# MuellerNico/DD2360-RayTracing

Measured on AMD Instinct MI355X. Metric: Msamples/s (W*H*spp/render_time) at 1200x800, 10000 spheres, higher is better.
Workload: dtype f32

## Files before the change

### dd2360-raytracing_amd/csrc/rt_kernels.hip

```cpp
#include <hip/hip_runtime.h>
#include <float.h>
#include "rt_device.h"
#include "rt_tuning.h"
#include "rt_sampling.h"

#ifdef RT_TU_CONTRACT
#pragma clang fp contract(fast)
#else
#pragma clang fp contract(off)
#endif

namespace rt {
#ifdef RT_TU_CONTRACT
namespace fmac {
#endif

#define RT_DEV static __device__ __forceinline__

#include "rt_stats.h"

struct Rng { uint32_t d, v0, v1, v2, v3, v4; };

RT_DEV float rng_uniform(Rng& s) {
    const uint32_t t = s.v0 ^ (s.v0 >> 2);
// ... 338 lines not shown
RT_DEV void walk_sync() { __builtin_amdgcn_fence(__ATOMIC_SEQ_CST, "wavefront"); __builtin_amdgcn_wave_barrier(); }
RT_DEV unsigned walk_excl_scan(unsigned v, unsigned& total) {
    int x = (int)v;
    x += __builtin_amdgcn_update_dpp(0, x, 0x111, 0xf, 0xf, false);
    x += __builtin_amdgcn_update_dpp(0, x, 0x112, 0xf, 0xf, false);
    x += __builtin_amdgcn_update_dpp(0, x, 0x114, 0xf, 0xf, false);
    x += __builtin_amdgcn_update_dpp(0, x, 0x118, 0xf, 0xf, false);
    x += __builtin_amdgcn_update_dpp(0, x, 0x142, 0xa, 0xf, false);
    x += __builtin_amdgcn_update_dpp(0, x, 0x143, 0xc, 0xf, false);
    total = (unsigned)__builtin_amdgcn_readlane(x, 63);
    return (unsigned)x - v;
}

RT_DEV void pool_candidate_b(const DevTree& T, const float4* s_nodes, WalkLds& L, const uint4 c, const float4 blo, const float4 bhi STAT_ARG) {
    const int owner = (int)c.w;
    const float b = __uint_as_float(c.x), disc = __uint_as_float(c.y);
    const float4 r0 = L.ray[2 * owner], r1 = L.ray[2 * owner + 1];
    RayF q; q.o = {r0.x, r0.y, r0.z}; q.d = {r0.w, r1.x, r1.y};
    const float a = r1.z;
    const unsigned long long k0 = L.key[owner];
    const float best_t = __uint_as_float((unsigned)(k0 >> 32));
    const int best = (int)(unsigned)k0;
    const float sq = sqrtf(disc);
    float cand = __builtin_inff();
    const float t1 = (-b - sq) / a;
    if (t1 > 0.001f) cand = t1;
    else { const float t2 = (-b + sq) / a; if (t2 > 0.001f) cand = t2; }
    if (!(cand <= best_t)) return;
    const int id = __float_as_int(blo.w);
    STAT(st, ST_OFFERS, 1);
// ... 45 lines not shown
    const float f_atm = a * (0.001f * 0.9999f - 1e-6f);
    bool walking = W.walking && W.i != W.iend;
    const int nw0 = __popcll(__ballot(walking));
    L.ray[2 * lane] = make_float4(r.o.x, r.o.y, r.o.z, r.d.x);
    while (true) {
        L.ray[2 * lane + 1] = make_float4(r.d.y, r.d.z, a, __builtin_fmaf(a * best_t, 1.0001f, 1e-6f * a));
        L.key[lane] = ((unsigned long long)__float_as_uint(best_t) << 32) | (unsigned)best;
        if (lane == 0) { L.tie_lo = 0u; L.tie_hi = 0u; }
        walk_sync();
        const int cols_now = nw0 * RT_POOL_COLS_THIN <= kWalkPool ? RT_POOL_COLS_THIN : RT_POOL_COLS;
        int e0[RT_POOL_COLS_THIN], e1[RT_POOL_COLS_THIN];
#pragma unroll
        for (int c = 0; c < RT_POOL_COLS_THIN; ++c) {
            e0[c] = 0; e1[c] = 0;
            if (c < cols_now && walking && W.i != W.iend) {
                STAT(st, ST_COLS, 1);
                const float u0 = W.on_c + ((float)W.i - W.om_c) * W.slope, u1 = u0 + W.slope;
                const float lo = (fminf(u0, u1) - q_c) * fF, hi = (fmaxf(u0, u1) + q_c) * fF;
                if (hi >= 0.0f && lo < fGf) {
                    const int k0 = (int)fmaxf(lo, 0.0f), k1 = (int)fminf(hi, fGfm);
                    const unsigned cbase = (unsigned)(W.coff + W.i * Gf);
                    e0[c] = cs[cbase + (unsigned)k0]; e1[c] = cs[cbase + (unsigned)k1 + 1u];
                }
                W.i += step; ++W.cols;
            }
        }
        unsigned n_seg = 0u;
#pragma unroll
        for (int c = 0; c < RT_POOL_COLS_THIN; ++c) {
            if (c >= RT_POOL_COLS && c >= cols_now) break;
            const bool has = e1[c] > e0[c];
// ... 35 lines not shown
                    S.sg = (n_seg > 1u && p1 <= begin ? 1u : 0u) + (n_seg > 2u && p2 <= begin ? 1u : 0u) + (n_seg > 3u && p3 <= begin ? 1u : 0u);
                } else if (begin < S.end) {
                    unsigned lo = 0u, hi = n_seg;
#pragma unroll
                    for (int it = 0; it < 8; ++it) {
                        const unsigned mid = (lo + hi) >> 1;
                        if (hi - lo > 1u) { if (L.pref[mid] <= begin) lo = mid; else hi = mid; }
                    }
                    S.sg = lo;
                }
            }
            unsigned qn = 0u;
            if (RT_POOL_DIRECT && RT_POOL_SPANS == 1 && total <= 64u) {
                PoolSpan& S = sp[0];
                const bool act = S.cur < S.end;
                STAT(st, ST_A_ITERS_WAVE, 1);
                unsigned he = 0u;
                if (act) {
                    const uint2 sd = L.seg[S.sg];
                    const unsigned p0 = L.pref[S.sg];
                    he = sd.x - p0 + S.cur;
                    S.owner = (int)(sd.y >> 26);
                    const float4 r0 = L.ray[2 * S.owner], r1 = L.ray[2 * S.owner + 1];
                    S.q.o = {r0.x, r0.y, r0.z}; S.q.d = {r0.w, r1.x, r1.y}; S.a = r1.z; S.abt = r1.w;
                    S.atm = S.a * (0.001f * 0.9999f - 1e-6f);
                }
                const float4 s4 = hot[he], blo = A.brick[2 * he], bhi = A.brick[2 * he + 1];
                STAT(st, ST_TESTS, act ? 1 : 0); STAT(st, ST_A_LANE_STEPS, act ? 1 : 0);
                const float ocx = S.q.o.x - s4.x, ocy = S.q.o.y - s4.y, ocz = S.q.o.z - s4.z;
                const float b = ocx * S.q.d.x + ocy * S.q.d.y + ocz * S.q.d.z;
                const float c = (ocx * ocx + ocy * ocy + ocz * ocz) - s4.w;
                const float disc = b * b - S.a * c;
                const float ab = fabsf(b);
                const float Lm = __builtin_fmaf(ab, -1e-4f, -b) - S.abt, M = __builtin_fmaf(ab, -1e-4f, b) + S.atm;
                const float P = fmaxf(Lm, M);
                if (act && disc > 0.0f && !(P > 0.0f && P * P > disc * 1.0003f)) {
                    STAT(st, ST_DISCPOS, 1);
                    pool_candidate_b(T, s_nodes, L, make_uint4(__float_as_uint(b), __float_as_uint(disc), he, (unsigned)S.owner), blo, bhi STAT_PASS);
                }
            } else
            while (true) {
                bool any = false;
#pragma unroll
                for (int j = 0; j < RT_POOL_SPANS; ++j) any = any || sp[j].cur < sp[j].end;
                if (__ballot(any) == 0ull) break;
                STAT(st, ST_A_ITERS_WAVE, 1);
                bool act[RT_POOL_SPANS]; unsigned he[RT_POOL_SPANS]; float4 s4[RT_POOL_SPANS];
#pragma unroll
                for (int j = 0; j < RT_POOL_SPANS; ++j) {
                    PoolSpan& S = sp[j];
                    act[j] = S.cur < S.end;
                    if (act[j] && S.cur >= S.seg_end) {
                        const uint2 sd = L.seg[S.sg];
                        const unsigned p0 = L.pref[S.sg];
                        ++S.sg;
                        S.seg_end = p0 + (sd.y & 0x3ffffffu);
                        S.base = sd.x - p0;
                        const int ow = (int)(sd.y >> 26);
                        if (ow != S.owner) {
                            S.owner = ow;
                            const float4 r0 = L.ray[2 * ow], r1 = L.ray[2 * ow + 1];
// ... 11 lines not shown
                    const PoolSpan& S = sp[j];
                    STAT(st, ST_TESTS, act[j] ? 1 : 0); STAT(st, ST_A_LANE_STEPS, act[j] ? 1 : 0);
                    const float ocx = S.q.o.x - s4[j].x, ocy = S.q.o.y - s4[j].y, ocz = S.q.o.z - s4[j].z;
                    const float b = ocx * S.q.d.x + ocy * S.q.d.y + ocz * S.q.d.z;
                    const float c = (ocx * ocx + ocy * ocy + ocz * ocz) - s4[j].w;
                    const float disc = b * b - S.a * c;
                    const float ab = fabsf(b);
                    const float Lm = __builtin_fmaf(ab, -1e-4f, -b) - S.abt, M = __builtin_fmaf(ab, -1e-4f, b) + S.atm;
                    const float P = fmaxf(Lm, M);
                    hold[j] = act[j] && disc > 0.0f && !(P > 0.0f && P * P > disc * 1.0003f);
                    hb[j] = b; hd[j] = disc;
                    anyhold = anyhold || hold[j];
                    if (act[j]) ++sp[j].cur;
                }
                if (__ballot(anyhold) != 0ull) {
#pragma unroll
                    for (int j = 0; j < RT_POOL_SPANS; ++j) {
                        const unsigned long long hm = __ballot(hold[j]);
                        if (hm != 0ull) {
                            const unsigned slot = qn + __builtin_amdgcn_mbcnt_hi((unsigned)(hm >> 32), __builtin_amdgcn_mbcnt_lo((unsigned)hm, 0u));
                            if (hold[j]) {
                                STAT(st, ST_DISCPOS, 1);
                                const uint4 ce = make_uint4(__float_as_uint(hb[j]), __float_as_uint(hd[j]), he[j], (unsigned)sp[j].owner);
                                if (slot < (unsigned)kWalkCand) L.cq[slot] = ce;
                                else pool_candidate(T, s_nodes, L, ce STAT_PASS);
                            }
                            qn += (unsigned)__popcll(hm);
                        }
                    }
                }
                if (qn >= 64u) pool_drain(T, s_nodes, L, lane, qn STAT_PASS);
            }
            pool_drain(T, s_nodes, L, lane, qn STAT_PASS);
            (void)f_atm;
            const unsigned long long k = L.key[lane];
            best_t = __uint_as_float((unsigned)(k >> 32)); best = (int)(unsigned)k;
            const unsigned tmask = lane < 32 ? L.tie_lo : L.tie_hi;
            if ((tmask >> (lane & 31)) & 1u) tie = true;
        }
        if (walking && best >= 0) walk_clip(W, A, best_t);
        walking = walking && W.i != W.iend;
        const int left = __popcll(__ballot(walking));
        if (left == 0) break;
        if (RT_QUORUM_DEN > 0 && nw0 >= RT_QUORUM_MIN && left * RT_QUORUM_DEN <= nw0) break;
    }
    W.walking = walking;
}

template <int RT_QUORUM_DEN>
RT_DEV void walk_pool_dense(const DevTree& T, const float4* s_nodes, WalkLds& L, const RayF& r, float a, Walk& W, float& best_t, int& best, bool& tie STAT_ARG) {
    constexpr int PB = RT_DENSE_PB;
    const DevAccel& A = T.acc;
    const int32_t* __restrict__ cs = A.cs;
    const float4* __restrict__ hot = A.hot;
    const int lane = threadIdx.x & 63;
    const int Gf = A.Gf;
    const float fF = (float)A.F, fGf = (float)Gf, fGfm = fGf - 0.5f, q_c = A.rq_c;
    const int step = W.fwd ? 1 : -1;
    bool walking = W.walking && W.i != W.iend;
    const int nw0 = __popcll(__ballot(walking));
    L.ray[2 * lane] = make_float4(r.o.x, r.o.y, r.o.z, r.d.x);
    while (true) {
        L.ray[2 * lane + 1] = make_float4(r.d.y, r.d.z, a, __builtin_fmaf(a * best_t, 1.0001f, 1e-6f * a));
        L.key[lane] = ((unsigned long long)__float_as_uint(best_t) << 32) | (unsigned)best;
        if (lane == 0) { L.tie_lo = 0u; L.tie_hi = 0u; }
        walk_sync();
        int e0 = 0, e1 = 0;
        if (walking && W.i != W.iend) {
            STAT(st, ST_COLS, 1);
            const float u0 = W.on_c + ((float)W.i - W.om_c) * W.slope, u1 = u0 + W.slope;
            const float lo = (fminf(u0, u1) - q_c) * fF, hi = (fmaxf(u0, u1) + q_c) * fF;
            if (hi >= 0.0f && lo < fGf) {
                const int k0 = (int)fmaxf(lo, 0.0f), k1 = (int)fminf(hi, fGfm);
                const unsigned cbase = (unsigned)(W.coff + W.i * Gf);
                e0 = cs[cbase + (unsigned)k0]; e1 = cs[cbase + (unsigned)k1 + 1u];
            }
            W.i += step; ++W.cols;
        }
        const bool has = e1 > e0;
        const unsigned long long m = __ballot(has);
        const unsigned n_seg = (unsigned)__popcll(m);
        if (has) {
            const unsigned slot = __builtin_amdgcn_mbcnt_hi((unsigned)(m >> 32), __builtin_amdgcn_mbcnt_lo((unsigned)m, 0u));
            L.seg[slot] = make_uint2((unsigned)e0, (unsigned)(e1 - e0) | ((unsigned)lane << 26));
// ... 14 lines not shown
            S.end = min(begin + C, total); S.cur = begin; S.seg_end = begin; S.base = 0u; S.sg = 0u; S.owner = lane;
            S.q.o = {0.f, 0.f, 0.f}; S.q.d = {0.f, 1.f, 0.f}; S.a = 1.0f; S.abt = 0.0f; S.atm = 0.0f;
            if (begin < S.end) {
                unsigned lo = 0u, hi = n_seg;
#pragma unroll
                for (int it = 0; it < 6; ++it) {
                    const unsigned mid = (lo + hi) >> 1;
                    if (hi - lo > 1u) { if (L.pref[mid] <= begin) lo = mid; else hi = mid; }
                }
                S.sg = lo;
            }
            unsigned qn = 0u;
            while (true) {
                const bool act = S.cur < S.end;
                if (__ballot(act) == 0ull) break;
                STAT(st, ST_A_ITERS_WAVE, 1);
                if (act && S.cur >= S.seg_end) {
                    const uint2 sd = L.seg[S.sg];
                    const unsigned p0 = L.pref[S.sg];
                    ++S.sg;
                    S.seg_end = p0 + (sd.y & 0x3ffffffu);
                    S.base = sd.x - p0;
                    S.owner = (int)(sd.y >> 26);
                    const float4 r0 = L.ray[2 * S.owner], r1 = L.ray[2 * S.owner + 1];
                    S.q.o = {r0.x, r0.y, r0.z}; S.q.d = {r0.w, r1.x, r1.y}; S.a = r1.z;
                    S.atm = S.a * (0.001f * 0.9999f - 1e-6f);
                }
                const unsigned nb = act ? min((unsigned)PB, min(S.seg_end, S.end) - S.cur) : 0u;
                const unsigned he0 = act ? S.base + S.cur : 0u;
                const float4* __restrict__ hp = hot + he0;
                float4 s4[PB];
// ... 6 lines not shown
                bool anyhold = false;
#pragma unroll
                for (int k = 0; k < PB; ++k) {
                    const float ocx = S.q.o.x - s4[k].x, ocy = S.q.o.y - s4[k].y, ocz = S.q.o.z - s4[k].z;
                    const float b = ocx * S.q.d.x + ocy * S.q.d.y + ocz * S.q.d.z;
                    const float c = (ocx * ocx + ocy * ocy + ocz * ocz) - s4[k].w;
                    const float disc = b * b - S.a * c;
                    const float ab = fabsf(b);
                    const float Lm = __builtin_fmaf(ab, -1e-4f, -b) - S.abt, M = __builtin_fmaf(ab, -1e-4f, b) + S.atm;
                    const float P = fmaxf(Lm, M);
                    hold[k] = (unsigned)k < nb && disc > 0.0f && !(P > 0.0f && P * P > disc * 1.0003f);
                    hb[k] = b; hd[k] = disc;
                    anyhold = anyhold || hold[k];
                }
                if (__ballot(anyhold) != 0ull) {
#pragma unroll
                    for (int k = 0; k < PB; ++k) {
                        const unsigned long long hm = __ballot(hold[k]);
                        if (hm != 0ull) {
                            const unsigned slot = qn + __builtin_amdgcn_mbcnt_hi((unsigned)(hm >> 32), __builtin_amdgcn_mbcnt_lo((unsigned)hm, 0u));
                            if (hold[k]) {
                                STAT(st, ST_DISCPOS, 1);
                                const uint4 ce = make_uint4(__float_as_uint(hb[k]), __float_as_uint(hd[k]), he0 + (unsigned)k, (unsigned)S.owner);
                                if (slot < (unsigned)kWalkCand) L.cq[slot] = ce;
                                else pool_candidate(T, s_nodes, L, ce STAT_PASS);
                            }
                            qn += (unsigned)__popcll(hm);
                        }
                    }
                }
                S.cur += nb;
                if (qn >= (unsigned)RT_DENSE_DRAIN) pool_drain(T, s_nodes, L, lane, qn STAT_PASS);
            }
            pool_drain(T, s_nodes, L, lane, qn STAT_PASS);
            const unsigned long long k = L.key[lane];
            best_t = __uint_as_float((unsigned)(k >> 32)); best = (int)(unsigned)k;
            const unsigned tmask = lane < 32 ? L.tie_lo : L.tie_hi;
            if ((tmask >> (lane & 31)) & 1u) tie = true;
        }
        if (walking && best >= 0) walk_clip(W, A, best_t);
        walking = walking && W.i != W.iend;
        const int left = __popcll(__ballot(walking));
        if (left == 0) break;
        if (RT_QUORUM_DEN > 0 && nw0 >= RT_QUORUM_MIN && left * RT_QUORUM_DEN <= nw0) break;
    }
    W.walking = walking;
}

constexpr int kHotLarge = 8;
constexpr int kHotSlots = 1 + 3 * kHotLarge;
RT_DEV float4* hot_spheres(const float4* s_nodes, int n_nodes) { return (float4*)((WalkLds*)(s_nodes + n_nodes * 3) + 4); }
template <bool POOL>
RT_DEV void stage_tree_fp32(const DevScene& S, const DevTree& T, float4* s_nodes) {
    const int n4 = T.n_nodes * 3;
    for (int t = threadIdx.x; t < n4; t += 256) s_nodes[t] = T.nodes4[t];
    if (POOL) {
        float4* h = hot_spheres(s_nodes, T.n_nodes);
        const int nl = min(T.acc.n_large, kHotLarge);
        if (threadIdx.x == 0) h[0] = S.ground_valid ? S.list_hot[0] : make_float4(0.f, 0.f, 0.f, 0.f);
        if ((int)threadIdx.x < nl) h[1 + threadIdx.x] = T.acc.large_hot[threadIdx.x];
        if ((int)threadIdx.x < 2 * nl) h[1 + kHotLarge + threadIdx.x] = T.acc.large_brick[threadIdx.x];
    }
    __syncthreads();
}

struct TreeState { Walk W; float g_t; int g_id; bool tie, pending; unsigned work, cols; };
RT_DEV void tree_state_init(TreeState& ts) {
    ts.pending = false; ts.tie = false; ts.g_t = FLT_MAX; ts.g_id = -1; ts.work = 0u; ts.cols = 0u; ts.W.work = 0u; ts.W.cols = 0u;
    ts.W.walking = false; ts.W.i = 0; ts.W.iend = 0; ts.W.coff = 0; ts.W.om_c = 0.f; ts.W.on_c = 0.f; ts.W.slope = 0.f; ts.W.dm_c = 0.f; ts.W.fwd = true;
}

template <int COOPG>
RT_DEV void closest_tree(const DevScene& S, const DevTree& T, const float4* s_nodes, const RayF& r, float a, bool live, float& closest, int& best, TreeState& ts STAT_ARG) {
    const bool fresh = live && !ts.pending;
    STAT(st, ST_RAYS, fresh ? 1 : 0);
    if (fresh) { closest = FLT_MAX; best = -1; }
    if (S.ground_valid && fresh) {
        WPASS(WP_GROUND);
        const float4 g = COOPG != 1 ? hot_spheres(s_nodes, T.n_nodes)[0] : S.list_hot[0];
        int gb = -1;
        { const float ocx = r.o.x - g.x, ocy = r.o.y - g.y, ocz = r.o.z - g.z;
          const float b = ocx * r.d.x + ocy * r.d.y + ocz * r.d.z;
          const float c = (ocx * ocx + ocy * ocy + ocz * ocz) - g.w;
          if (__ballot(fresh && !(b > 0.0f && c > 0.0f)) != 0ull) sphere_test(r, a, g.x, g.y, g.z, g.w, 0, closest, gb); }
// ... 54 lines not shown
        }
        if (walker) {
            ts.pending = ts.W.walking;
            if (!ts.pending && ts.tie) { closest = ts.g_t; best = ts.g_id; slow = true; STAT(st, ST_TIE, 1); }
        }
    }
    RT_STATS_ONLY(
    const unsigned long long tS0 = TICK(); st.cyc[1] += tS0 - tG;
    )
    if (__ballot(slow) != 0ull) { WPASS(WP_SCAN); tree_scan(s_nodes, r, a, slow, closest, best); }
    RT_STATS_ONLY(
    st.cyc[3] += TICK() - tS0;
    )
}

RT_DEV V3 random_in_unit_sphere(Rng& s) {
    V3 p;
    do {
        WPASS(WP_REJ_ITER);
        const float x = rng_uniform(s); const float y = rng_uniform(s); const float z = rng_uniform(s);
        p.x = signed_unit(x); p.y = signed_unit(y); p.z = signed_unit(z);
    } while (p.x * p.x + p.y * p.y + p.z * p.z >= 1.0f);
    return p;
}

RT_DEV RayF primary_ray(const rt_camera& c, int i, int j, int max_x, int max_y, Rng& s) {
    const float u = ((float)i + rng_uniform(s)) / (float)max_x;
    const float v = ((float)j + rng_uniform(s)) / (float)max_y;
    float px, py;
    WPASS(WP_PRIMARY);
// ... 272 lines not shown
            fb[0] = (float)pix_iters; fb[1] = (float)((__builtin_amdgcn_s_memrealtime() >> 4) & 0xffffffull); fb[2] = (float)((pix_t0 >> 4) & 0xffffffull);
            )
        } else {
            if (A.ns == 1) { fb[0] = col.x; fb[1] = col.y; fb[2] = col.z; }
            else { fb[0] += col.x; fb[1] += col.y; fb[2] += col.z; }
        }
    };
    RT_STATS_ONLY(
    Stats st; for (int q = 0; q < ST_N; ++q) st.c[q] = 0;
    for (int q = 0; q < 8; ++q) st.cyc[q] = 0;
    const unsigned long long tK0 = TICK(), rK0 = __builtin_amdgcn_s_memrealtime();
    unsigned int dbg_thin_iters = 0, dbg_long = 0;
    unsigned long long th[4] = {0, 0, 0, 0};
    unsigned long long dbg_thin_cyc = 0, dbg_thin_closest = 0, dbg_thin1_cyc = 0; unsigned int dbg_thin1_iters = 0; unsigned long long dbg_t_prev = TICK();
    )
    constexpr bool kSolo = TREE && COOPG == 5;
    if (kSolo && lane == 0 && begin_long_pixel(true)) solo = true;
    if (__ballot(live) == 0ull && lane < RT_LONG_PER_WAVE) begin_long_pixel(false);
    if (__ballot(live) != 0ull) { thin = true; __builtin_amdgcn_s_setprio(3); }

    const unsigned int thin_cap = (unsigned int)(n_waves / RT_THIN_CAP_DEN);
    float closest = FLT_MAX; int best = -1;
    TreeState ts; tree_state_init(ts);
    while (true) {
        const unsigned long long m_live = __ballot(live);
        const unsigned long long m_long = __ballot(live && is_long);
        if (!thin && m_long != 0ull) {
            unsigned int prev = 0;
            if (lane == 0) prev = atomicAdd(cold_args()->queue + 1, 1u);
            prev = __builtin_amdgcn_readfirstlane(prev);
            if (prev < thin_cap) { thin = true; thin_counted = true; __builtin_amdgcn_s_setprio(3); }
            else { if (lane == 0) atomicSub(cold_args()->queue + 1, 1u); is_long = false; }
        } else if (thin && m_long == 0ull) {
// ... 29 lines not shown
        { const unsigned long long now = TICK(); const int nl2 = __popcll(__ballot(live));
          if (thin) { ++dbg_thin_iters; dbg_thin_cyc += now - dbg_t_prev; if (nl2 <= 2) { ++dbg_thin1_iters; dbg_thin1_cyc += now - dbg_t_prev; } }
          dbg_t_prev = now; }
        )
        RT_STATS_ONLY(
        { const int nl = __popcll(__ballot(live)); STAT(st, nl >= 56 ? ST_LIVE_GE56 : nl >= 32 ? ST_LIVE_32 : nl >= 8 ? ST_LIVE_8 : ST_LIVE_LT8, 1);
          WPASS_CLASS(nl >= 56 ? 0 : nl >= 32 ? 1 : nl >= 8 ? 2 : 3); }
        )
        const float a = dot3(r.d, r.d);
        if (!TREE) { closest = FLT_MAX; best = -1; }
        RT_STATS_ONLY(
        const unsigned long long tC0 = TICK();
        const unsigned long long c4_ = st.cyc[4], c5_ = st.cyc[5], c1_ = st.cyc[1], c3_ = st.cyc[3];
        const bool thin12 = thin && __popcll(__ballot(live)) <= 2;
        )
        if (TREE) closest_tree<COOPG>(A.scene, A.tree, s_nodes, r, a, live, closest, best, ts STAT_PASS);
        else closest_list(A.scene, r, a, live, closest, best);
        RT_STATS_ONLY(
        const unsigned long long tC1 = TICK(); st.cyc[0] += tC1 - tC0; st.cyc[2] += tC0; if (thin) dbg_thin_closest += tC1 - tC0;
        if (TREE && thin12) { th[0] += (st.cyc[4] - c4_) - tC0; th[1] += st.cyc[5] - c5_; th[2] += (st.cyc[1] - c1_) - (st.cyc[5] - c5_); th[3] += st.cyc[3] - c3_; }
        if (live) { ++pix_iters; }
        )
        if (live && !(TREE && ts.pending)) {
            ++iters;
            bool done;
            float lum = 0.0f;
            if (best >= 0) {
                const bool cont = scatter(cold_args()->scene, best, closest, r, att, s);
                ++depth;
                done = !cont || depth >= 50;
            } else {
// ... 18 lines not shown
                        RT_STATS_ONLY(
                        if (!is_long) ++dbg_long;
                        )
                        is_long = true;
                    }
                    else if (RT_MED_RATE > 0 && (sample & 7) == 0 && iters >= (unsigned int)(RT_MED_RATE * sample)) is_med = true;
                } else {
                    WPASS(WP_ENDPIX);
                    end_pixel();
                    RT_STATS_ONLY(
                    pix_iters = 0;
                    )
                    STAT(st, ST_SWITCHES, 1);
                    live = false; is_long = false; is_med = false;
                    if (kSolo && solo && begin_long_pixel(true)) {  }
                    else if (lane < RT_LONG_PER_WAVE && begin_long_pixel(false)) { solo = false;  }
                }
            }
        }
    }

    RT_STATS_ONLY(
    for (int q = 0; q < ST_N; ++q) {
        const bool wave_level = (q == ST_LOOP_ITERS_WAVE || (q >= ST_LIVE_GE56 && q <= ST_LIVE_LT8));
        const bool lane_max = (q == ST_A_ITERS_WAVE || q == ST_B_ROUNDS_WAVE);
        if (lane_max) { int m = (int)st.c[q]; for (int off = 32; off > 0; off >>= 1) m = max(m, __shfl_xor(m, off)); if (lane == 0) atomicAdd(&g_stats[q], (unsigned long long)m); }
        else if (st.c[q] && (!wave_level || lane == 0)) atomicAdd(&g_stats[q], (unsigned long long)st.c[q]);
    }
    { int nl = (int)dbg_long; for (int off = 32; off > 0; off >>= 1) nl += __shfl_xor(nl, off); dbg_long = (unsigned int)nl; }
    if (lane == 0) {
        const long long wv = (long long)blockIdx.x * 4 + (threadIdx.x >> 6);
// ... 401 lines not shown
    const unsigned int mine = s_bin[threadIdx.x];
    s_base[threadIdx.x] = mine != 0u ? start + atomicAdd(&ws[256 + threadIdx.x], mine) : 0u;
    __syncthreads();
#pragma unroll
    for (int u = 0; u < 4; ++u) {
        if (key[u] < 0) continue;
        const int sub = (int)((b0 + 256 * u + threadIdx.x) & 15);
        const unsigned int pos = s_base[key[u]] + local[u];
        const int lx = 2 * (sub & 3), ly = 2 * (sub >> 2);
#pragma unroll
        for (int q = 0; q < 4; ++q) tail_list[pos + q] = (unsigned int)(tile[u] * 64 + (ly + (q >> 1)) * 8 + lx + (q & 1));
    }
}
#endif

template <bool TREE, int COOPG>
RT_DEV void trace_record(const RenderArgs& A, const float4* s_nodes, const RayF& r, bool live, rt_hit_record* out) {
    const DevScene& S = A.scene; const DevTree& T = A.tree;
    const float a = dot3(r.d, r.d);
    float closest = FLT_MAX; int best = -1;
    RT_STATS_ONLY(
    Stats st; for (int q = 0; q < ST_N; ++q) st.c[q] = 0;
    for (int q = 0; q < 8; ++q) st.cyc[q] = 0;
    )
    if (TREE) {
        TreeState ts; tree_state_init(ts);
        bool act = live;
        do { closest_tree<COOPG>(S, T, s_nodes, r, a, act, closest, best, ts STAT_PASS); act = live && ts.pending; } while (__ballot(act) != 0ull);
    } else closest_list(S, r, a, live, closest, best);
    if (!live) return;
    rt_hit_record h;
    h.sphere = best; h.t = 0.f; h.p[0] = h.p[1] = h.p[2] = 0.f; h.normal[0] = h.normal[1] = h.normal[2] = 0.f;
    if (best >= 0) {
        const float4 g = S.geom[best];
        h.t = closest;
        h.p[0] = r.o.x + closest * r.d.x; h.p[1] = r.o.y + closest * r.d.y; h.p[2] = r.o.z + closest * r.d.z;
        h.normal[0] = (h.p[0] - g.x) / g.w; h.normal[1] = (h.p[1] - g.y) / g.w; h.normal[2] = (h.p[2] - g.z) / g.w;
    }
    *out = h;
}

template <bool TREE, int COOPG = 1>
__global__ __launch_bounds__(256) void k_trace(RenderArgs A, const float* rays, long long n, rt_hit_record* out) {
    extern __shared__ float4 s_nodes[];
    if (TREE) stage_tree_fp32<COOPG != 1>(A.scene, A.tree, s_nodes);
    const long long gid = (long long)blockIdx.x * 256 + threadIdx.x;
    const bool live = gid < n;
    RayF r; r.o = {0.f, 0.f, 0.f}; r.d = {0.f, 1.f, 0.f};
    if (live) { const float* p = rays + gid * 6; r.o = {p[0], p[1], p[2]}; r.d = {p[3], p[4], p[5]}; }
    trace_record<TREE, COOPG>(A, s_nodes, r, live, out + gid);
}

#ifndef RT_TU_CONTRACT
template <bool TREE, int COOPG = 1>
__global__ __launch_bounds__(256) void k_guides(RenderArgs A, long long n, rt_hit_record* out) {
    extern __shared__ float4 s_nodes[];
    if (TREE) stage_tree_fp32<COOPG != 1>(A.scene, A.tree, s_nodes);
    const long long gid = (long long)blockIdx.x * 256 + threadIdx.x;
    const bool live = gid < n;
    RayF r; r.o = {0.f, 0.f, 0.f}; r.d = {0.f, 1.f, 0.f};
    if (live) {
        const rt_camera& c = A.scene.cam;
        const int i = (int)(gid % A.max_x), j = (int)(gid / A.max_x);
        const float u = ((float)i + 0.5f) / (float)A.max_x;
        const float v = ((float)j + 0.5f) / (float)A.max_y;
// ... 267 lines not shown
    return hipGetLastError();
}
hipError_t launch_adapt_zero(unsigned int* p, int n, hipStream_t st) {
    if (n <= 0) return hipSuccess;
    hipLaunchKernelGGL(k_adapt_zero, dim3((unsigned)((n + 255) / 256)), dim3(256), 0, st, p, n);
    return hipGetLastError();
}
#endif

hipError_t launch_trace(const DevScene& S, const DevTree& T, bool tree, const float* rays, long long n, rt_hit_record* out, hipStream_t st) {
    if (n <= 0) return hipSuccess;
    const unsigned blocks = (unsigned)((n + 255) / 256);
    RenderArgs A{};
    A.scene = S; A.tree = T;
    if (!tree) return launch_trace_list(A, blocks, rays, n, out, st);
    if (render_variant(true, 0, T.acc) == 5) hipLaunchKernelGGL((k_trace<true, 5>), dim3(blocks), dim3(256), tree_lds_bytes(T.n_nodes, true), st, A, rays, n, out);
    else if (render_variant(true, 0, T.acc) == 4) hipLaunchKernelGGL((k_trace<true, 4>), dim3(blocks), dim3(256), tree_lds_bytes(T.n_nodes, true), st, A, rays, n, out);
    else if (render_variant(true, 0, T.acc) == 2) hipLaunchKernelGGL((k_trace<true, 2>), dim3(blocks), dim3(256), tree_lds_bytes(T.n_nodes, true), st, A, rays, n, out);
    else hipLaunchKernelGGL((k_trace<true>), dim3(blocks), dim3(256), tree_lds_bytes(T.n_nodes), st, A, rays, n, out);
    return hipGetLastError();
}

#ifndef RT_TU_CONTRACT
hipError_t launch_guides(const DevScene& S, const DevTree& T, bool tree, int max_x, int max_y, rt_hit_record* out, hipStream_t st) {
    const long long n = (long long)max_x * max_y;
    if (n <= 0) return hipSuccess;
    const unsigned blocks = (unsigned)((n + 255) / 256);
    RenderArgs A{};
    A.scene = S; A.tree = T; A.max_x = max_x; A.max_y = max_y;
    if (!tree) return launch_guides_list(A, blocks, n, out, st);
// ... 34 lines not shown
```

### dd2360-raytracing_amd/csrc/rt_stats.h

```cpp
#pragma once
#ifdef RT_STATS
enum { ST_RAYS, ST_FAST, ST_SLOW, ST_TIE, ST_COLS, ST_TESTS, ST_DISCPOS, ST_OFFERS, ST_ELIG, ST_ELIG_NODES, ST_A_ITERS_WAVE, ST_B_ROUNDS_WAVE,
       ST_LOOP_ITERS_WAVE, ST_A_LANE_STEPS, ST_B_LANES, ST_SAMPLES, ST_LIVE_GE56, ST_LIVE_32, ST_LIVE_8, ST_LIVE_LT8, ST_SWITCHES,
       ST_CYC_TOTAL, ST_CYC_CLOSEST, ST_CYC_WALK_A, ST_CYC_WALK_B, ST_CYC_SCAN, ST_CYC_SHADE, ST_REALTIME,
       ST_SPARE0, ST_SPARE1, ST_SPARE2, ST_SPARE3, ST_SPARE4, ST_SPARE5, ST_SPARE6,
       WP_GROUND, WP_LARGE_K, WP_LARGE_EXACT, WP_OFFER_NODE, WP_OFFER_RAYBOX, WP_ELIG_FN, WP_ELIG_LIST, WP_SETUP, WP_A_COL, WP_A_BATCH, WP_A_HOLD,
       WP_B_OFFER, WP_B_CLIP, WP_COOP_CHUNK, WP_SCAN, WP_SC_ANY, WP_SC_LAMB, WP_SC_METAL, WP_SC_DIEL, WP_REJ_ITER, WP_PRIMARY, WP_DISK_ITER, WP_SKY, WP_ENDPIX,
       TH_GROUND, TH_LARGE_SETUP, TH_WALK, TH_SCAN, ST_N };
#ifdef RT_STATS_LIGHT
#define TICK() 0ull
#else
#define TICK() ((unsigned long long)__builtin_amdgcn_s_memtime())
#endif
__device__ unsigned long long g_stats[ST_N];
__device__ int g_pilot_dbg[1 << 20];
__device__ unsigned long long g_wave_dbg[8192 * 4];
struct Stats { unsigned int c[ST_N]; unsigned long long cyc[8]; };
#ifdef RT_STATS_LIGHT
#define STAT(st, k, v) ((void)0)
#else
#define STAT(st, k, v) ((st).c[k] += (v))
#endif
constexpr int kWpBlocks = WP_ENDPIX - WP_GROUND + 1;
__device__ unsigned long long g_wp_cls[4 * kWpBlocks];
#ifdef RT_STATS_WPASS
__shared__ int s_wp_cls[4];
#define WPASS(k) do { const int l_ = (int)(threadIdx.x & 63); if (__builtin_amdgcn_readfirstlane(l_) == l_) { atomicAdd(&g_stats[k], 1ull); \
    atomicAdd(&g_wp_cls[(s_wp_cls[(threadIdx.x >> 6) & 3] & 3) * kWpBlocks + ((k) - WP_GROUND)], 1ull); } } while (0)
#define WPASS_CLASS(c) do { const int l_ = (int)(threadIdx.x & 63); if (__builtin_amdgcn_readfirstlane(l_) == l_) s_wp_cls[(threadIdx.x >> 6) & 3] = (c); } while (0)
#else
#define WPASS(k) ((void)0)
#define WPASS_CLASS(c) ((void)0)
#endif
#define STAT_ARG , Stats& st
#define STAT_PASS , st
#define RT_STATS_ONLY(...) __VA_ARGS__
#define RT_STATS_READERS \
hipError_t read_pilot_dbg(int* out, int n) { return hipMemcpyFromSymbol(out, HIP_SYMBOL(g_pilot_dbg), sizeof(int) * (size_t)(n < (1 << 20) ? n : (1 << 20))); } \
hipError_t read_wave_dbg(unsigned long long* out) { return hipMemcpyFromSymbol(out, HIP_SYMBOL(g_wave_dbg), sizeof(unsigned long long) * 8192 * 4); } \
hipError_t read_wp_classes(unsigned long long* out, int reset) { \
    hipError_t e = hipMemcpyFromSymbol(out, HIP_SYMBOL(g_wp_cls), sizeof(unsigned long long) * 4 * kWpBlocks); \
    if (e != hipSuccess) return e; \
    if (reset) { unsigned long long z[4 * kWpBlocks] = {0}; e = hipMemcpyToSymbol(HIP_SYMBOL(g_wp_cls), z, sizeof(z)); } \
// ... 18 lines not shown
```

### dd2360-raytracing_amd/csrc/rt_tuning.h

```cpp
#pragma once

#ifndef RT_RENDER_WAVES
#define RT_RENDER_WAVES 4
#endif

#ifndef RT_LONG_RATE
#define RT_LONG_RATE 14
#endif
#ifndef RT_LONG_RATE_DENSE
#define RT_LONG_RATE_DENSE 20
#endif
#ifndef RT_LONG_CHECK
#define RT_LONG_CHECK 4
#endif
#ifndef RT_F_INFLIGHT
#define RT_F_INFLIGHT 1.35f
#endif
#ifndef RT_F_INFLIGHT_DENSE
#define RT_F_INFLIGHT_DENSE 1.1f
#endif

#ifndef RT_F_STATIC
#define RT_F_STATIC 1.07f
#endif
// ... 20 lines not shown
#endif
#ifndef RT_LONG_RATE_MIN
#define RT_LONG_RATE_MIN 8
#endif
#ifndef RT_PILOT_LONG_SUM_MIN
#define RT_PILOT_LONG_SUM_MIN 120
#endif
#ifndef RT_MED_RATE
#define RT_MED_RATE 12
#endif
#ifndef RT_THIN_CAP_DEN
#define RT_THIN_CAP_DEN 4
#endif
#ifndef RT_LONG_PER_WAVE
#define RT_LONG_PER_WAVE 16
#endif
#ifndef RT_PILOT_SAMPLES
#define RT_PILOT_SAMPLES 2
#endif
#ifndef RT_PILOT_LONG_SUM
#define RT_PILOT_LONG_SUM 200
#endif
#ifndef RT_SOLO_DENSITY
#define RT_SOLO_DENSITY 1.0
#endif
#ifndef RT_PILOT_SOLO_SUM
#define RT_PILOT_SOLO_SUM 200
#endif
#ifndef RT_PILOT_CAP
#define RT_PILOT_CAP 35
// ... 97 lines not shown
```

Baseline: 4592.

## Add quad-lane cooperative ground and large-sphere tests for sparse long-pixel waves

When a wave has at most 16 live rays, all on lanes that are multiples of four, each ray's three idle neighbour lanes now test the ground and the first three large spheres in parallel, and the results are reduced with DPP quad broadcasts. Long-pixel chains are placed on lanes 0,4,...,60 so this layout arises in the render kernel, and a small-batch trace kernel uses it too. The aim is to cut the serial per-ray large-sphere loop in thin, divergent tail waves. The cost is extra DPP traffic, a redo fallback when a candidate lies outside its brick, and different lane placement of long chains, which could hurt walk-pool packing.

```diff
diff --git a/dd2360-raytracing_amd/csrc/rt_kernels.hip b/dd2360-raytracing_amd/csrc/rt_kernels.hip
--- a/dd2360-raytracing_amd/csrc/rt_kernels.hip
+++ b/dd2360-raytracing_amd/csrc/rt_kernels.hip
@@ -376,6 +376,7 @@
 
 RT_DEV void pool_candidate_b(const DevTree& T, const float4* s_nodes, WalkLds& L, const uint4 c, const float4 blo, const float4 bhi STAT_ARG) {
     const int owner = (int)c.w;
+    WPASS(WP_B_OFFER);
     const float b = __uint_as_float(c.x), disc = __uint_as_float(c.y);
     const float4 r0 = L.ray[2 * owner], r1 = L.ray[2 * owner + 1];
     RayF q; q.o = {r0.x, r0.y, r0.z}; q.d = {r0.w, r1.x, r1.y};
@@ -451,7 +452,7 @@
         for (int c = 0; c < RT_POOL_COLS_THIN; ++c) {
             e0[c] = 0; e1[c] = 0;
             if (c < cols_now && walking && W.i != W.iend) {
-                STAT(st, ST_COLS, 1);
+                STAT(st, ST_COLS, 1); WPASS(WP_A_COL);
                 const float u0 = W.on_c + ((float)W.i - W.om_c) * W.slope, u1 = u0 + W.slope;
                 const float lo = (fminf(u0, u1) - q_c) * fF, hi = (fmaxf(u0, u1) + q_c) * fF;
                 if (hi >= 0.0f && lo < fGf) {
@@ -517,7 +518,7 @@
             if (RT_POOL_DIRECT && RT_POOL_SPANS == 1 && total <= 64u) {
                 PoolSpan& S = sp[0];
                 const bool act = S.cur < S.end;
-                STAT(st, ST_A_ITERS_WAVE, 1);
+                STAT(st, ST_A_ITERS_WAVE, 1); WPASS(WP_COOP_CHUNK);
                 unsigned he = 0u;
                 if (act) {
                     const uint2 sd = L.seg[S.sg];
@@ -547,7 +548,7 @@
 #pragma unroll
                 for (int j = 0; j < RT_POOL_SPANS; ++j) any = any || sp[j].cur < sp[j].end;
                 if (__ballot(any) == 0ull) break;
-                STAT(st, ST_A_ITERS_WAVE, 1);
+                STAT(st, ST_A_ITERS_WAVE, 1); WPASS(WP_A_BATCH);
                 bool act[RT_POOL_SPANS]; unsigned he[RT_POOL_SPANS]; float4 s4[RT_POOL_SPANS];
 #pragma unroll
                 for (int j = 0; j < RT_POOL_SPANS; ++j) {
@@ -589,6 +590,7 @@
                     if (act[j]) ++sp[j].cur;
                 }
                 if (__ballot(anyhold) != 0ull) {
+                    WPASS(WP_A_HOLD);
 #pragma unroll
                     for (int j = 0; j < RT_POOL_SPANS; ++j) {
                         const unsigned long long hm = __ballot(hold[j]);
@@ -613,7 +615,7 @@
             const unsigned tmask = lane < 32 ? L.tie_lo : L.tie_hi;
             if ((tmask >> (lane & 31)) & 1u) tie = true;
         }
-        if (walking && best >= 0) walk_clip(W, A, best_t);
+        if (walking && best >= 0) { WPASS(WP_B_CLIP); walk_clip(W, A, best_t); }
         walking = walking && W.i != W.iend;
         const int left = __popcll(__ballot(walking));
         if (left == 0) break;
@@ -642,7 +644,7 @@
         walk_sync();
         int e0 = 0, e1 = 0;
         if (walking && W.i != W.iend) {
-            STAT(st, ST_COLS, 1);
+            STAT(st, ST_COLS, 1); WPASS(WP_A_COL);
             const float u0 = W.on_c + ((float)W.i - W.om_c) * W.slope, u1 = u0 + W.slope;
             const float lo = (fminf(u0, u1) - q_c) * fF, hi = (fmaxf(u0, u1) + q_c) * fF;
             if (hi >= 0.0f && lo < fGf) {
@@ -687,7 +689,7 @@
             while (true) {
                 const bool act = S.cur < S.end;
                 if (__ballot(act) == 0ull) break;
-                STAT(st, ST_A_ITERS_WAVE, 1);
+                STAT(st, ST_A_ITERS_WAVE, 1); WPASS(WP_A_BATCH);
                 if (act && S.cur >= S.seg_end) {
                     const uint2 sd = L.seg[S.sg];
                     const unsigned p0 = L.pref[S.sg];
@@ -724,6 +726,7 @@
                     anyhold = anyhold || hold[k];
                 }
                 if (__ballot(anyhold) != 0ull) {
+                    WPASS(WP_A_HOLD);
 #pragma unroll
                     for (int k = 0; k < PB; ++k) {
                         const unsigned long long hm = __ballot(hold[k]);
@@ -748,7 +751,7 @@
             const unsigned tmask = lane < 32 ? L.tie_lo : L.tie_hi;
             if ((tmask >> (lane & 31)) & 1u) tie = true;
         }
-        if (walking && best >= 0) walk_clip(W, A, best_t);
+        if (walking && best >= 0) { WPASS(WP_B_CLIP); walk_clip(W, A, best_t); }
         walking = walking && W.i != W.iend;
         const int left = __popcll(__ballot(walking));
         if (left == 0) break;
@@ -758,6 +761,7 @@
 }
 
 constexpr int kHotLarge = 8;
+constexpr int kQuadLarge = 3;
 constexpr int kHotSlots = 1 + 3 * kHotLarge;
 RT_DEV float4* hot_spheres(const float4* s_nodes, int n_nodes) { return (float4*)((WalkLds*)(s_nodes + n_nodes * 3) + 4); }
 template <bool POOL>
@@ -778,6 +782,42 @@
 RT_DEV void tree_state_init(TreeState& ts) {
     ts.pending = false; ts.tie = false; ts.g_t = FLT_MAX; ts.g_id = -1; ts.work = 0u; ts.cols = 0u; ts.W.work = 0u; ts.W.cols = 0u;
     ts.W.walking = false; ts.W.i = 0; ts.W.iend = 0; ts.W.coff = 0; ts.W.om_c = 0.f; ts.W.on_c = 0.f; ts.W.slope = 0.f; ts.W.dm_c = 0.f; ts.W.fwd = true;
+}
+
+RT_DEV bool quad_form(unsigned long long m_live) {
+    return RT_QUAD_MAX_LIVE > 0 && (m_live & ~0x1111111111111111ull) == 0ull && (int)__popcll(m_live) <= RT_QUAD_MAX_LIVE;
+}
+template <int CTRL> RT_DEV float quad_get(float v) { return __int_as_float(__builtin_amdgcn_update_dpp(0, __float_as_int(v), CTRL, 0xf, 0xf, false)); }
+template <int CTRL> RT_DEV int quad_get(int v) { return __builtin_amdgcn_update_dpp(0, v, CTRL, 0xf, 0xf, false); }
+constexpr int kQuad0 = 0x00, kQuad1 = 0x55, kQuad2 = 0xaa, kQuad3 = 0xff;
+
+RT_DEV bool quad_spheres(const DevTree& T, const float4* s_nodes, const RayF& r, float a, bool fresh, bool fast, float& closest, int& best, TreeState& ts) {
+    const int sub = threadIdx.x & 3;
+    RayF q;
+    q.o.x = quad_get<kQuad0>(r.o.x); q.o.y = quad_get<kQuad0>(r.o.y); q.o.z = quad_get<kQuad0>(r.o.z);
+    q.d.x = quad_get<kQuad0>(r.d.x); q.d.y = quad_get<kQuad0>(r.d.y); q.d.z = quad_get<kQuad0>(r.d.z);
+    const float qa = quad_get<kQuad0>(a);
+    const float4* hs = hot_spheres(s_nodes, T.n_nodes);
+    const int kl = sub > 0 ? sub - 1 : 0;
+    const float4 sp = hs[sub];
+    const float4 blo = hs[1 + kHotLarge + 2 * kl], bhi = hs[2 + kHotLarge + 2 * kl];
+    float cand = sphere_candidate(q, qa, sp);
+    if (sub > 0 && kl >= T.acc.n_large) cand = __builtin_inff();
+    const int info = __float_as_int(blo.w) | (in_brick(q, cand, blo, bhi) ? 0x40000000 : 0);
+    const float c1 = quad_get<kQuad1>(cand), c2 = quad_get<kQuad2>(cand), c3 = quad_get<kQuad3>(cand);
+    const int i1 = quad_get<kQuad1>(info), i2 = quad_get<kQuad2>(info), i3 = quad_get<kQuad3>(info);
+    const bool gh = cand < FLT_MAX;
+    const float g_t = gh ? cand : FLT_MAX; const int g_id = gh ? 0 : -1;
+    float bt = g_t; int bi = g_id; bool tie = false, redo = false;
+#define RT_QUAD_OFFER(c, i) { const int id = (i) & 0x3fffffff; \
+        if ((c) < bt) { if ((i) & 0x40000000) { bt = (c); bi = id; } else redo = true; } \
+        else if ((c) == bt && id != bi && bi > 0) tie = true; }
+    RT_QUAD_OFFER(c1, i1) RT_QUAD_OFFER(c2, i2) RT_QUAD_OFFER(c3, i3)
+#undef RT_QUAD_OFFER
+    if (__ballot(fresh && fast && redo) != 0ull) return false;
+    if (fresh) { closest = g_t; best = g_id; }
+    if (fresh && fast) { ts.g_t = g_t; ts.g_id = g_id; ts.tie = tie; closest = bt; best = bi; }
+    return true;
 }
 
 template <int COOPG>
@@ -862,6 +902,101 @@
     )
 }
 
+template <int COOPG>
+RT_DEV void closest_tree_quad(const DevScene& S, const DevTree& T, const float4* s_nodes, const RayF& r, float a, bool live, float& closest, int& best, TreeState& ts STAT_ARG) {
+    const bool fresh = live && !ts.pending;
+    STAT(st, ST_RAYS, fresh ? 1 : 0);
+    if (fresh) { closest = FLT_MAX; best = -1; }
+    auto is_fast = [&]() {
+        const float zx = r.o.x, zy = r.o.y - 1.0f, zz = r.o.z;
+        return fresh && (a >= 9.094947e-13f) && (a <= 1.0995116e12f) && (r.d.x != 0.0f) && (r.d.z != 0.0f)
+               && (fabsf(r.d.y) >= 9.094947e-13f) && (zx * zx + zy * zy + zz * zz <= T.acc.zone2);
+    };
+    bool fast = false;
+    bool quad = false;
+    {
+        if (S.ground_valid && T.acc.enabled && quad_form(__ballot(live)) && __ballot(fresh) != 0ull) {
+            WPASS(WP_QUAD);
+            fast = is_fast();
+            quad = quad_spheres(T, s_nodes, r, a, fresh, fast, closest, best, ts);
+            if (!quad) WPASS(WP_QUAD_REDO);
+        }
+    }
+    if (S.ground_valid && fresh && !quad) {
+        WPASS(WP_GROUND);
+        const float4 g = COOPG != 1 ? hot_spheres(s_nodes, T.n_nodes)[0] : S.list_hot[0];
+        int gb = -1;
+        { const float ocx = r.o.x - g.x, ocy = r.o.y - g.y, ocz = r.o.z - g.z;
+          const float b = ocx * r.d.x + ocy * r.d.y + ocz * r.d.z;
+          const float c = (ocx * ocx + ocy * ocy + ocz * ocz) - g.w;
+          if (__ballot(fresh && !(b > 0.0f && c > 0.0f)) != 0ull) sphere_test(r, a, g.x, g.y, g.z, g.w, 0, closest, gb); }
+        if (gb == 0) best = 0;
+    }
+    RT_STATS_ONLY(
+    const unsigned long long tG = TICK(); st.cyc[4] += tG;
+    )
+    bool slow = fresh;
+    if (COOPG != 1 && T.acc.enabled) {
+        if (!quad) fast = is_fast();
+        slow = fresh && !fast;
+        STAT(st, ST_FAST, fast ? 1 : 0); STAT(st, ST_SLOW, slow ? 1 : 0);
+        if (fast) {
+            if (!quad) { ts.g_t = closest; ts.g_id = best; ts.tie = false; }
+            const float ra = __builtin_amdgcn_rcpf(a);
+            for (int k = quad ? kQuadLarge : 0; k < T.acc.n_large; ++k) {
+                const float4* hs = hot_spheres(s_nodes, T.n_nodes);
+                const float4 sp = k < kHotLarge ? hs[1 + k] : T.acc.large_hot[k];
+                WPASS(WP_LARGE_K);
+                const float ocx = r.o.x - sp.x, ocy = r.o.y - sp.y, ocz = r.o.z - sp.z;
+                const float b = ocx * r.d.x + ocy * r.d.y + ocz * r.d.z;
+                const float c = (ocx * ocx + ocy * ocy + ocz * ocz) - sp.w;
+                const float disc = b * b - a * c;
+                if (disc > 0.0f) {
+                    const float sqa = __builtin_amdgcn_sqrtf(disc);
+                    const float m = 1e-4f * ((fabsf(b) + sqa) * ra) + 1e-6f;
+                    const bool behind = (sqa - b) * ra + m < 0.001f;
+                    const bool beyond = (-b - sqa) * ra - m > closest;
+                    if (!behind && !beyond) {
+                        WPASS(WP_LARGE_EXACT);
+                        const float sq = sqrtf(disc);
+                        float cand = __builtin_inff();
+                        const float t1 = (-b - sq) / a;
+                        if (t1 > 0.001f) cand = t1;
+                        else { const float t2 = (-b + sq) / a; if (t2 > 0.001f) cand = t2; }
+                        offer(T, s_nodes, r, cand, k < kHotLarge ? hs[1 + kHotLarge + 2 * k] : T.acc.large_brick[2 * k], k < kHotLarge ? hs[2 + kHotLarge + 2 * k] : T.acc.large_brick[2 * k + 1], closest, best, ts.tie STAT_PASS);
+                    }
+                }
+            }
+            WPASS(WP_SETUP);
+            ts.W = walk_setup(T.acc, r, closest, best);
+        }
+        RT_STATS_ONLY(
+        const unsigned long long tL = TICK(); st.cyc[5] += tL - tG;
+        )
+        const bool walker = fast || (live && ts.pending);
+        const int nw = __popcll(__ballot(walker));
+        if (nw > 0) {
+            WalkLds& L = *((WalkLds*)(s_nodes + T.n_nodes * 3) + (threadIdx.x >> 6));
+            Walk Wl = ts.W; Wl.walking = walker && ts.W.walking;
+            float bt = walker ? closest : FLT_MAX; int bi = walker ? best : -1; bool tt = false;
+            if (COOPG >= 4) walk_pool<RT_QUORUM_SPARSE>(T, s_nodes, L, r, a, Wl, bt, bi, tt STAT_PASS);
+            else walk_pool_dense<RT_QUORUM_DENSE>(T, s_nodes, L, r, a, Wl, bt, bi, tt STAT_PASS);
+            if (walker) { ts.work += Wl.work; ts.cols += Wl.cols; Wl.work = 0u; Wl.cols = 0u; ts.W = Wl; closest = bt; best = bi; ts.tie = ts.tie || tt; }
+        }
+        if (walker) {
+            ts.pending = ts.W.walking;
+            if (!ts.pending && ts.tie) { closest = ts.g_t; best = ts.g_id; slow = true; STAT(st, ST_TIE, 1); }
+        }
+    }
+    RT_STATS_ONLY(
+    const unsigned long long tS0 = TICK(); st.cyc[1] += tS0 - tG;
+    )
+    if (__ballot(slow) != 0ull) { WPASS(WP_SCAN); tree_scan(s_nodes, r, a, slow, closest, best); }
+    RT_STATS_ONLY(
+    st.cyc[3] += TICK() - tS0;
+    )
+}
+
 RT_DEV V3 random_in_unit_sphere(Rng& s) {
     V3 p;
     do {
@@ -1164,9 +1299,12 @@
     unsigned long long th[4] = {0, 0, 0, 0};
     unsigned long long dbg_thin_cyc = 0, dbg_thin_closest = 0, dbg_thin1_cyc = 0; unsigned int dbg_thin1_iters = 0; unsigned long long dbg_t_prev = TICK();
     )
+    constexpr bool kQuad = TREE && COOPG == 4 && MODE != 1 && RT_QUAD_MAX_LIVE > 0;
+    static_assert(!kQuad || RT_LONG_PER_WAVE <= 16, "with the quad form the long lanes are 0, 4, ..., 60: at most 16 chains a wave");
+    const bool quad_long_lane = (lane & 3) == 0 && (lane >> 2) < RT_LONG_PER_WAVE;
     constexpr bool kSolo = TREE && COOPG == 5;
     if (kSolo && lane == 0 && begin_long_pixel(true)) solo = true;
-    if (__ballot(live) == 0ull && lane < RT_LONG_PER_WAVE) begin_long_pixel(false);
+    if (__ballot(live) == 0ull && (kQuad ? quad_long_lane : lane < RT_LONG_PER_WAVE)) begin_long_pixel(false);
     if (__ballot(live) != 0ull) { thin = true; __builtin_amdgcn_s_setprio(3); }
 
     const unsigned int thin_cap = (unsigned int)(n_waves / RT_THIN_CAP_DEN);
@@ -1226,7 +1364,8 @@
         const unsigned long long c4_ = st.cyc[4], c5_ = st.cyc[5], c1_ = st.cyc[1], c3_ = st.cyc[3];
         const bool thin12 = thin && __popcll(__ballot(live)) <= 2;
         )
-        if (TREE) closest_tree<COOPG>(A.scene, A.tree, s_nodes, r, a, live, closest, best, ts STAT_PASS);
+        if constexpr (kQuad) closest_tree_quad<COOPG>(A.scene, A.tree, s_nodes, r, a, live, closest, best, ts STAT_PASS);
+        else if (TREE) closest_tree<COOPG>(A.scene, A.tree, s_nodes, r, a, live, closest, best, ts STAT_PASS);
         else closest_list(A.scene, r, a, live, closest, best);
         RT_STATS_ONLY(
         const unsigned long long tC1 = TICK(); st.cyc[0] += tC1 - tC0; st.cyc[2] += tC0; if (thin) dbg_thin_closest += tC1 - tC0;
@@ -1275,7 +1414,7 @@
                     STAT(st, ST_SWITCHES, 1);
                     live = false; is_long = false; is_med = false;
                     if (kSolo && solo && begin_long_pixel(true)) {  }
-                    else if (lane < RT_LONG_PER_WAVE && begin_long_pixel(false)) { solo = false;  }
+                    else if ((kQuad ? quad_long_lane : lane < RT_LONG_PER_WAVE) && begin_long_pixel(false)) { solo = false;  }
                 }
             }
         }
@@ -1707,7 +1846,7 @@
 }
 #endif
 
-template <bool TREE, int COOPG>
+template <bool TREE, int COOPG, bool QUAD = false>
 RT_DEV void trace_record(const RenderArgs& A, const float4* s_nodes, const RayF& r, bool live, rt_hit_record* out) {
     const DevScene& S = A.scene; const DevTree& T = A.tree;
     const float a = dot3(r.d, r.d);
@@ -1719,6 +1858,8 @@
     if (TREE) {
         TreeState ts; tree_state_init(ts);
         bool act = live;
+        if constexpr (QUAD) { do { closest_tree_quad<COOPG>(S, T, s_nodes, r, a, act, closest, best, ts STAT_PASS); act = live && ts.pending; } while (__ballot(act) != 0ull); }
+        else
         do { closest_tree<COOPG>(S, T, s_nodes, r, a, act, closest, best, ts STAT_PASS); act = live && ts.pending; } while (__ballot(act) != 0ull);
     } else closest_list(S, r, a, live, closest, best);
     if (!live) return;
@@ -1742,6 +1883,16 @@
     RayF r; r.o = {0.f, 0.f, 0.f}; r.d = {0.f, 1.f, 0.f};
     if (live) { const float* p = rays + gid * 6; r.o = {p[0], p[1], p[2]}; r.d = {p[3], p[4], p[5]}; }
     trace_record<TREE, COOPG>(A, s_nodes, r, live, out + gid);
+}
+template <int COOPG>
+__global__ __launch_bounds__(256) void k_trace_quad(RenderArgs A, const float* rays, long long n, rt_hit_record* out) {
+    extern __shared__ float4 s_nodes[];
+    stage_tree_fp32<true>(A.scene, A.tree, s_nodes);
+    const long long gid = threadIdx.x >> 2;
+    const bool live = threadIdx.x < 64 && (threadIdx.x & 3) == 0 && gid < n;
+    RayF r; r.o = {0.f, 0.f, 0.f}; r.d = {0.f, 1.f, 0.f};
+    if (live) { const float* p = rays + gid * 6; r.o = {p[0], p[1], p[2]}; r.d = {p[3], p[4], p[5]}; }
+    trace_record<true, COOPG, true>(A, s_nodes, r, live, out + gid);
 }
 
 #ifndef RT_TU_CONTRACT
@@ -2039,6 +2190,13 @@
     RenderArgs A{};
     A.scene = S; A.tree = T;
     if (!tree) return launch_trace_list(A, blocks, rays, n, out, st);
+    const int variant = render_variant(true, 0, T.acc);
+    if (RT_QUAD_MAX_LIVE > 0 && n <= 16 && n <= RT_QUAD_MAX_LIVE && variant != 1) {
+        if (variant == 5) hipLaunchKernelGGL((k_trace_quad<5>), dim3(1), dim3(256), tree_lds_bytes(T.n_nodes, true), st, A, rays, n, out);
+        else if (variant == 4) hipLaunchKernelGGL((k_trace_quad<4>), dim3(1), dim3(256), tree_lds_bytes(T.n_nodes, true), st, A, rays, n, out);
+        else hipLaunchKernelGGL((k_trace_quad<2>), dim3(1), dim3(256), tree_lds_bytes(T.n_nodes, true), st, A, rays, n, out);
+        return hipGetLastError();
+    }
     if (render_variant(true, 0, T.acc) == 5) hipLaunchKernelGGL((k_trace<true, 5>), dim3(blocks), dim3(256), tree_lds_bytes(T.n_nodes, true), st, A, rays, n, out);
     else if (render_variant(true, 0, T.acc) == 4) hipLaunchKernelGGL((k_trace<true, 4>), dim3(blocks), dim3(256), tree_lds_bytes(T.n_nodes, true), st, A, rays, n, out);
     else if (render_variant(true, 0, T.acc) == 2) hipLaunchKernelGGL((k_trace<true, 2>), dim3(blocks), dim3(256), tree_lds_bytes(T.n_nodes, true), st, A, rays, n, out);
diff --git a/dd2360-raytracing_amd/csrc/rt_stats.h b/dd2360-raytracing_amd/csrc/rt_stats.h
--- a/dd2360-raytracing_amd/csrc/rt_stats.h
+++ b/dd2360-raytracing_amd/csrc/rt_stats.h
@@ -6,7 +6,8 @@
        ST_SPARE0, ST_SPARE1, ST_SPARE2, ST_SPARE3, ST_SPARE4, ST_SPARE5, ST_SPARE6,
        WP_GROUND, WP_LARGE_K, WP_LARGE_EXACT, WP_OFFER_NODE, WP_OFFER_RAYBOX, WP_ELIG_FN, WP_ELIG_LIST, WP_SETUP, WP_A_COL, WP_A_BATCH, WP_A_HOLD,
        WP_B_OFFER, WP_B_CLIP, WP_COOP_CHUNK, WP_SCAN, WP_SC_ANY, WP_SC_LAMB, WP_SC_METAL, WP_SC_DIEL, WP_REJ_ITER, WP_PRIMARY, WP_DISK_ITER, WP_SKY, WP_ENDPIX,
-       TH_GROUND, TH_LARGE_SETUP, TH_WALK, TH_SCAN, ST_N };
+       TH_GROUND, TH_LARGE_SETUP, TH_WALK, TH_SCAN,
+       WP_QUAD, WP_QUAD_REDO, ST_N };
 #ifdef RT_STATS_LIGHT
 #define TICK() 0ull
 #else
@@ -21,12 +22,14 @@
 #else
 #define STAT(st, k, v) ((st).c[k] += (v))
 #endif
-constexpr int kWpBlocks = WP_ENDPIX - WP_GROUND + 1;
+constexpr int kWpFirst = WP_ENDPIX - WP_GROUND + 1;
+constexpr int kWpBlocks = kWpFirst + 2;
+#define WP_SLOT(k) ((k) >= WP_QUAD ? (k) - WP_QUAD + kWpFirst : (k) - WP_GROUND)
 __device__ unsigned long long g_wp_cls[4 * kWpBlocks];
 #ifdef RT_STATS_WPASS
 __shared__ int s_wp_cls[4];
 #define WPASS(k) do { const int l_ = (int)(threadIdx.x & 63); if (__builtin_amdgcn_readfirstlane(l_) == l_) { atomicAdd(&g_stats[k], 1ull); \
-    atomicAdd(&g_wp_cls[(s_wp_cls[(threadIdx.x >> 6) & 3] & 3) * kWpBlocks + ((k) - WP_GROUND)], 1ull); } } while (0)
+    atomicAdd(&g_wp_cls[(s_wp_cls[(threadIdx.x >> 6) & 3] & 3) * kWpBlocks + WP_SLOT(k)], 1ull); } } while (0)
 #define WPASS_CLASS(c) do { const int l_ = (int)(threadIdx.x & 63); if (__builtin_amdgcn_readfirstlane(l_) == l_) s_wp_cls[(threadIdx.x >> 6) & 3] = (c); } while (0)
 #else
 #define WPASS(k) ((void)0)
diff --git a/dd2360-raytracing_amd/csrc/rt_tuning.h b/dd2360-raytracing_amd/csrc/rt_tuning.h
--- a/dd2360-raytracing_amd/csrc/rt_tuning.h
+++ b/dd2360-raytracing_amd/csrc/rt_tuning.h
@@ -58,6 +58,9 @@
 #endif
 #ifndef RT_LONG_PER_WAVE
 #define RT_LONG_PER_WAVE 16
+#endif
+#ifndef RT_QUAD_MAX_LIVE
+#define RT_QUAD_MAX_LIVE 16
 #endif
 #ifndef RT_PILOT_SAMPLES
 #define RT_PILOT_SAMPLES 2
```

Measured after the change: 4675, median of 6. 1.02x the previous value.
